# Sahar-E/NeRF-and-DietNeRF

Measured on AMD Instinct MI355X. Metric: rays/sec (coarse+fine) at 256x256, 64 coarse + 128 fine samples, higher is better.
Workload: dtype f16 (3-pass hi/lo split operands, f32 accumulate; fp32-class results)

## Files before the change

### include/nerf_mi355.h

```cpp
#ifndef NERF_MI355_H
#define NERF_MI355_H

#include <stddef.h>
#include <stdint.h>

#ifdef __cplusplus
extern "C" {
#endif

#define NERF_ABI_VERSION 6

enum { NERF_NET_COARSE = 0, NERF_NET_FINE = 1 };
enum { NERF_MEM_HOST = 0, NERF_MEM_DEVICE = 1 };
enum {
    NERF_PRECISION_FP32 = 0,
    NERF_PRECISION_F16X3 = 1,
    NERF_PRECISION_F16 = 2,
    NERF_PRECISION_BF16X3 = 3
};

enum {
    NERF_SAMPLING_LINEAR = 0,
    NERF_SAMPLING_LINDISP = 1
};
// ... 135 lines not shown
int nerf_train_render_gradients(nerf_ctx* ctx, const float* rays_orig, const float* rays_dirs, const float* d_rgb,
                                int64_t N, int32_t Sc, int32_t Sf, const float* u_coarse, const float* u_fine,
                                uint64_t seed, int64_t ray_base, int32_t accumulate, float* rgb_out,
                                float* grad_coarse, float* grad_fine, int mem);
int nerf_train_render_forward(nerf_ctx* ctx, int32_t slot, const float* rays_orig, const float* rays_dirs, int64_t N,
                              int32_t Sc, int32_t Sf, const float* u_coarse, const float* u_fine, uint64_t seed,
                              int64_t ray_base, float* rgb_out, int mem);
int nerf_train_render_backward(nerf_ctx* ctx, int32_t slot, const float* d_rgb, int32_t accumulate, float* grad_coarse,
                               float* grad_fine, int mem);
int nerf_train_render_release(nerf_ctx* ctx);
int nerf_train_get_gradients(nerf_ctx* ctx, int which, float* blob, size_t n_floats, int mem);
int nerf_get_weights(nerf_ctx* ctx, int which, float* blob, size_t n_floats, int mem);

int nerf_ctx_enable_timing(nerf_ctx* ctx, int on);
int nerf_ctx_read_timing(nerf_ctx* ctx, double* mlp_ms, int64_t* n_launches, int64_t* n_rows);
int nerf_ctx_read_culling_timing(nerf_ctx* ctx, double* ms4, int64_t* n_passes);

#ifdef __cplusplus
}
#endif
#endif
```

### nerf_and_dietnerf_amd/_lib.py

```python
from __future__ import annotations

import ctypes as C
import os

_HERE = os.path.dirname(os.path.abspath(__file__))
LIB_PATH = os.environ.get("NERF_MI355_LIB") or os.path.join(_HERE, "lib", "libnerf_mi355.so")

NERF_NET_COARSE, NERF_NET_FINE = 0, 1
NERF_MEM_HOST, NERF_MEM_DEVICE = 0, 1
NERF_PRECISION_FP32, NERF_PRECISION_F16X3, NERF_PRECISION_F16, NERF_PRECISION_BF16X3 = 0, 1, 2, 3
NERF_SAMPLING_LINEAR, NERF_SAMPLING_LINDISP = 0, 1
NERF_RAYS_WORLD, NERF_RAYS_NDC = 0, 1
NERF_ABI_VERSION = 6


class NerfConfig(C.Structure):
    _fields_ = [
        ("n_pos_enc_xyz", C.c_int32), ("n_pos_enc_dir", C.c_int32), ("n_angles", C.c_int32),
        ("hidden_dim", C.c_int32), ("last_hidden_dim", C.c_int32), ("leaky_relu_alpha", C.c_float),
        ("near_boundary", C.c_float), ("far_boundary", C.c_float), ("precision", C.c_int32),
        ("device", C.c_int32),
    ]


# ... 65 lines not shown
    ("nerf_train_set_distortion_weights", C.c_int, [_P, _F, _F]),
    ("nerf_train_read_distortion_sums", C.c_int, [_P, C.POINTER(C.c_double), C.POINTER(_I64)]),
    ("nerf_distortion_loss", C.c_int, [_P, _P, _P, _I64, _I32, _P, _P, _P, C.c_int]),
    ("nerf_train_loss_scale", C.c_int, [_P, C.POINTER(C.c_float), C.POINTER(_I64), C.POINTER(_I64)]),
    ("nerf_train_read_metric_sums", C.c_int, [_P, C.POINTER(C.c_double), C.POINTER(_I64)]),
    ("nerf_train_step", C.c_int, [_P, _P, _P, _P, _I64, _I32, _I32, _P, _P, _U64, _P, C.c_int]),
    ("nerf_train_gradients", C.c_int, [_P, _P, _P, _P, _I64, _I32, _I32, _P, _P, _U64, _P, _P, _P, C.c_int]),
    ("nerf_train_apply", C.c_int, [_P, _P, _P, C.c_int]),
    ("nerf_train_render_gradients", C.c_int, [_P, _P, _P, _P, _I64, _I32, _I32, _P, _P, _U64, _I64, _I32, _P, _P, _P,
                                              C.c_int]),
    ("nerf_train_render_forward", C.c_int, [_P, _I32, _P, _P, _I64, _I32, _I32, _P, _P, _U64, _I64, _P, C.c_int]),
    ("nerf_train_render_backward", C.c_int, [_P, _I32, _P, _I32, _P, _P, C.c_int]),
    ("nerf_train_render_release", C.c_int, [_P]),
    ("nerf_train_get_gradients", C.c_int, [_P, C.c_int, _P, C.c_size_t, C.c_int]),
    ("nerf_get_weights", C.c_int, [_P, C.c_int, _P, C.c_size_t, C.c_int]),
    ("nerf_ctx_enable_timing", C.c_int, [_P, C.c_int]),
    ("nerf_ctx_read_timing", C.c_int, [_P, C.POINTER(C.c_double), C.POINTER(_I64), C.POINTER(_I64)]),
]

_lib = None


def load():
    global _lib
    if _lib is not None:
        return _lib
    if not os.path.exists(LIB_PATH):
        raise RuntimeError(
            f"{LIB_PATH} is missing: build the HIP extension first "
            "(python -c 'import __graft_entry__ as g; g.build()' or make -C nerf_and_dietnerf_amd/csrc). "
# ... 24 lines not shown
```

### nerf_and_dietnerf_amd/csrc/mlp_f16x3.hip

```cpp
#include "mlp_f16_frag.h"

#include <math.h>
#include <string.h>

#if defined(NERF_BF16) && NERF_PE_LX == 5
namespace nerf::bf16 {
#elif defined(NERF_BF16)
namespace nerf::bf16::wide {
#elif NERF_PE_LX == 5
namespace nerf {
#else
namespace nerf::wide {
#endif

#ifdef NERF_BF16
typedef __bf16 e8 __attribute__((ext_vector_type(8)));
typedef __bf16 bf2 __attribute__((ext_vector_type(2)));
#define NERF_MFMA_E16 __builtin_amdgcn_mfma_f32_32x32x16_bf16
__device__ __forceinline__ void split_e(float y, float& hi_f, float& lo_f) {
    hi_f = __uint_as_float(__float_as_uint(y) & 0xFFFF0000u);
    lo_f = y - hi_f;
}
__device__ __forceinline__ uint32_t pack_hi(float a, float b) {
    return __builtin_amdgcn_perm(__float_as_uint(b), __float_as_uint(a), 0x07060302u);
// ... 318 lines not shown
    constexpr bool kPPBuild = false;
#else
    constexpr bool kPPBuild = true;
#endif
    constexpr bool kPP = kPPBuild && !FAST && !STASH && !XYZ;
    extern __shared__ __attribute__((aligned(16))) char smem[];
    const int tid = threadIdx.x;
    const int lane = tid & 63;
    const int wave = __builtin_amdgcn_readfirstlane(tid >> 6);
    const int j = lane & 31;
    const int h = lane >> 5;
    const uint32_t lane16 = kLdsRing + lane * 16;
    uint32_t cb_h = kLdsConst + h * 16;
    asm volatile("" : "+v"(cb_h));

    const long long ntiles = (a.M + 127) / 128;
    if ((long long)blockIdx.x >= ntiles) return;

    for (int i = tid; i < (XYZ ? kXConstFloats : kHConstFloats) / 4; i += 256) {
        const bool sig = SIGONLY && i >= kHConstBias8 / 4 && i < (kHConstBias8 + 32) / 4;
        reinterpret_cast<f32x4*>(smem + kLdsConst)[i] =
            reinterpret_cast<const f32x4*>(a.wconst)[sig ? i + (kHConstBiasSig - kHConstBias8) / 4 : i];
    }

    Pipe p;
    p.ck = 0;
    p.src_next = 0;
    p.n_chunks = XYZ ? (FAST ? kXFStreamChunks : kXStreamChunks) : SIGONLY ? kHStreamChunksSig : (FAST ? kFStreamChunks : kHStreamChunks);
    p.wbase = reinterpret_cast<const char*>(a.wstream);
    p.voff = wave * (kHCQ / 4 * kQuadBytes) + lane * 16;
    p.wave_lds = wave * (kHCQ / 4 * kQuadBytes);
    __syncthreads();
// ... 4 lines not shown
        p.src_next += 1;
#pragma unroll
        for (int j = 0; j < kHCQ / 4; ++j) dma_piece(p.cur_src, p.voff + j * kQuadBytes, p.cur_dst + j * kQuadBytes);
    }
    asm volatile("s_waitcnt vmcnt(%0)" ::"n"((kHCQ / 4) * (kHRing - 2)) : "memory");
    __builtin_amdgcn_s_barrier();
    asm volatile("" ::: "memory");

    frag4 xh[16], xl[16], nh[kPP ? 16 : 14], nl[kPP ? 16 : 14], peh[kHStepsPE], pel[kHStepsPE], dh[2], dl[2];
    f32x16 accs[4];
    float xc[64];
    float sigma_raw = 0.f;

    unsigned long long t0 = 0, t1 = 0, acc_t[8] = {0, 0, 0, 0, 0, 0, 0, 0};
    (void)t0; (void)t1; (void)acc_t;
    for (long long tile = blockIdx.x; tile < ntiles; tile += gridDim.x) {
        STAMP(t0);
        const long long m = tile * 128 + wave * 32 + j;
        const bool valid = m < a.M;
        const long long mm = valid ? m : a.M - 1;
        float px, py, pz, dx, dy, dz;
        if (a.mode == 0) {
            const long long ray = mm / a.S;
            const f32x4 o = *reinterpret_cast<const f32x4*>(a.in_a + ray * 4);
            const f32x4 d = *reinterpret_cast<const f32x4*>(a.in_b + ray * 4);
            const float zz = a.z[mm];
            px = __fadd_rn(o[0], __fmul_rn(d[0], zz));
            py = __fadd_rn(o[1], __fmul_rn(d[1], zz));
            pz = __fadd_rn(o[2], __fmul_rn(d[2], zz));
            dx = d[0]; dy = d[1]; dz = d[2];
        } else {
            px = a.in_a[mm * 3 + 0]; py = a.in_a[mm * 3 + 1]; pz = a.in_a[mm * 3 + 2];
            if constexpr (XYZ) { dx = dy = dz = 0.f; }
            else { dx = a.in_b[mm * 3 + 0]; dy = a.in_b[mm * 3 + 1]; dz = a.in_b[mm * 3 + 2]; }
        }
        const float kPi = 3.1415927410125732f;
        float pv[8 * kHStepsPE];
#pragma unroll
        for (int c = 0; c < 3; ++c) {
            const float v = c == 0 ? px : c == 1 ? py : pz;
            if constexpr (FAST) {
                sin_ladder_fp16_modes<kPeLx>(v * kPi, h, &pv[c * kPeLx]);
            } else {
#pragma unroll
                for (int k = 0; k < kPeLx; ++k) pv[c * kPeLx + k] = sin_shifted(v * (kPi * (float)(1 << k)), h);
            }
        }
        if constexpr (kPeLx == 5) {
            pv[15] = h ? 0.f : px; pv[16] = h ? 0.f : py; pv[17] = h ? 0.f : pz;
#pragma unroll
            for (int i = 18; i < 24; ++i) pv[i] = 0.f;
        } else {
            static_assert(kPeLx == 10, "the wide-PE layout holds exactly 10 octaves");
            pv[30] = h ? pz : px; pv[31] = h ? 0.f : py;
        }
#pragma unroll
        for (int n = 0; n < kHStepsPE; ++n) {
            float t8[8];
#pragma unroll
            for (int e = 0; e < 8; ++e) t8[e] = pv[n * 8 + e];
            split8<FAST>(t8, peh[n], pel[n]);
        }
        float dv[16];
#pragma unroll
        for (int c = 0; c < 3; ++c) {
            const float v = c == 0 ? dx : c == 1 ? dy : dz;
            if constexpr (FAST) {
                sin_ladder_fp16_modes<kLd>(v * kPi, h, &dv[c * kLd]);
            } else {
#pragma unroll
                for (int k = 0; k < kLd; ++k) dv[c * kLd + k] = sin_shifted(v * (kPi * (float)(1 << k)), h);
            }
        }
#pragma unroll
        for (int i = 12; i < 16; ++i) dv[i] = 0.f;
#pragma unroll
        for (int n = 0; n < 2; ++n) {
            float t8[8];
#pragma unroll
            for (int e = 0; e < 8; ++e) t8[e] = dv[n * 8 + e];
            split8<FAST>(t8, dh[n], dl[n]);
        }

        auto st_of = [&](int l) -> float* {
            if constexpr (!STASH) return nullptr;
            else {
                const long long row0 = a.diag_wrap ? (long long)(blockIdx.x & 63) * 128 + wave * 32 : tile * 128 + wave * 32;
                const long long off = row0 * (long long)a.st_ld[l] + (h * 32 + j) * 4;
                if constexpr (FAST) return reinterpret_cast<float*>(reinterpret_cast<uint16_t*>(a.st_ptr[l]) + off);
                else return a.st_ptr[l] + off;
            }
        };
        auto mk_of = [&](int l) -> frag4* {
            if constexpr (!STASH) return nullptr;
            else return a.mask_ptr[l] ? reinterpret_cast<frag4*>(a.mask_ptr[l]) + (tile * 128 + wave * 32 + j) * 2 + h
                                      : nullptr;
// ... 51 lines not shown
        } else {
            st_prev = st_cur;
            st_cur = st_of(8);
            mk_prev_ptr = mk_cur_ptr; mk_cur_ptr = mk_of(8);
            mk_prev = mk_cur; mk_cur = frag4{0u, 0u, 0u, 0u};
            if constexpr (kPP) layer_body_h<BODY_LAST, true, FAST, STASH, 0, true>(p, lane16, cb_h, kHConstBias8 * 4, a.alpha, st_prev, st_cur, mk_prev_ptr, mk_cur_ptr, mk_prev, mk_cur, accs, nh, nl, xh, xl, peh, pel, dh, dl, xc, sigma_raw);
            else layer_body_h<BODY_LAST, true, FAST, STASH>(p, lane16, cb_h, kHConstBias8 * 4, a.alpha, st_prev, st_cur, mk_prev_ptr, mk_cur_ptr, mk_prev, mk_cur, accs, xh, xl, nh, nl, peh, pel, dh, dl, xc, sigma_raw);
            STAMP(t1); acc_t[4] += t1 - t0;
        }
        if constexpr (SIGONLY) {
            if (valid && h == 0) {
                a.raw[m] = sigma_raw;
                if (a.nonfinite && !(fabsf(sigma_raw) <= 3.0e38f)) atomicAdd(a.nonfinite, 1ull);
            }
            STAMP(t0); acc_t[5] += t0 - t1; acc_t[6] += 1;
            continue;
        }
        float o0 = 0.f, o1 = 0.f, o2 = 0.f;
#pragma unroll
        for (int t = 0; t < 4; ++t) {
#pragma unroll
            for (int g = 0; g < 4; ++g) {
                constexpr int kW = XYZ ? kXConstWrgb : kHConstWrgb;
                const f32x4 w0 = lds_read4(cb_h + (kW + 0 * 128 + t * 32 + g * 8) * 4);
                const f32x4 w1 = lds_read4(cb_h + (kW + 1 * 128 + t * 32 + g * 8) * 4);
                const f32x4 w2 = lds_read4(cb_h + (kW + 2 * 128 + t * 32 + g * 8) * 4);
#pragma unroll
                for (int e = 0; e < 4; ++e) {
                    const float x = xc[t * 16 + g * 4 + e];
                    o0 = fmaf(w0[e], x, o0);
// ... 2 lines not shown
                }
            }
        }
        o0 += __shfl_xor(o0, 32);
        o1 += __shfl_xor(o1, 32);
        o2 += __shfl_xor(o2, 32);
        const f32x4 bh = lds_read4(kLdsConst + (XYZ ? kXConstBHead : kHConstBHead) * 4);
        if (valid && h == 0) {
            f32x4 out;
            out[0] = o0 + bh[0]; out[1] = o1 + bh[1]; out[2] = o2 + bh[2]; out[3] = sigma_raw;
            *reinterpret_cast<f32x4*>(a.raw + m * 4) = out;
            const float chk = out[0] + out[1] + out[2] + out[3];
            if (a.nonfinite && !(fabsf(chk) <= 3.0e38f)) atomicAdd(a.nonfinite, 1ull);
        }
        STAMP(t0); acc_t[5] += t0 - t1; acc_t[6] += 1;
    }
#ifdef NERF_STAMPS
    if (blockIdx.x == 0 && tid == 0)
        for (int i = 0; i < 8; ++i) g_stamps_h[i] = acc_t[i];
#endif
    asm volatile("s_waitcnt vmcnt(0)" ::: "memory");
}

#ifdef NERF_BF16
__global__ __launch_bounds__(256, 1) void mlp_bf16x3_kernel(const MlpArgs a) { mlp_f16_body<false>(a); }
__global__ __launch_bounds__(256, 1) void mlp_bf16x3_xyz_kernel(const MlpArgs a) { mlp_f16_body<false, false, true>(a); }
#if NERF_PE_LX == 5
__global__ __launch_bounds__(256, 1) void mlp_bf16x3_sig_kernel(const MlpArgs a) { mlp_f16_body<false, false, false, true>(a); }
#endif

// ... 36 lines not shown
__global__ __launch_bounds__(256, 1) void mlp_f16_xyz_stash_kernel(const MlpArgs a) { mlp_f16_body<true, true, true>(a); }

void launch_mlp_f16x3_stash(const MlpArgs& a, int num_cus, hipStream_t stream, bool single_pass, bool xyz_only) {
    if (a.M <= 0) return;
    const long long ntiles = (a.M + 127) / 128;
    const int grid = (int)(ntiles < (long long)num_cus ? ntiles : (long long)num_cus);
    if (xyz_only) {
        if (single_pass) hipLaunchKernelGGL(mlp_f16_xyz_stash_kernel, dim3(grid), dim3(256), kLdsTotal, stream, a);
        else hipLaunchKernelGGL(mlp_f16x3_xyz_stash_kernel, dim3(grid), dim3(256), kLdsTotal, stream, a);
        return;
    }
    if (single_pass) hipLaunchKernelGGL(mlp_f16_stash_kernel, dim3(grid), dim3(256), kLdsTotal, stream, a);
    else hipLaunchKernelGGL(mlp_f16x3_stash_kernel, dim3(grid), dim3(256), kLdsTotal, stream, a);
}

void launch_mlp_f16x3(const MlpArgs& a, int num_cus, hipStream_t stream, bool single_pass, bool xyz_only) {
    if (a.M <= 0) return;
    const long long ntiles = (a.M + 127) / 128;
    const int grid = (int)(ntiles < (long long)num_cus ? ntiles : (long long)num_cus);
    if (xyz_only) {
        if (single_pass) hipLaunchKernelGGL(mlp_f16_xyz_kernel, dim3(grid), dim3(256), kLdsTotal, stream, a);
        else hipLaunchKernelGGL(mlp_f16x3_xyz_kernel, dim3(grid), dim3(256), kLdsTotal, stream, a);
        return;
    }
    if (single_pass) hipLaunchKernelGGL(mlp_f16_kernel, dim3(grid), dim3(256), kLdsTotal, stream, a);
    else hipLaunchKernelGGL(mlp_f16x3_kernel, dim3(grid), dim3(256), kLdsTotal, stream, a);
}

#if NERF_PE_LX == 5
void launch_mlp_f16x3_sig(const MlpArgs& a, int num_cus, hipStream_t stream) {
    if (a.M <= 0) return;
    const long long ntiles = (a.M + 127) / 128;
    const int grid = (int)(ntiles < (long long)num_cus ? ntiles : (long long)num_cus);
    hipLaunchKernelGGL(mlp_f16x3_sig_kernel, dim3(grid), dim3(256), kLdsTotal, stream, a);
}
#endif

#if defined(NERF_STAMPS) && NERF_PE_LX == 5
extern "C" void nerf_debug_read_stamps_h(unsigned long long* out) {
    (void)hipDeviceSynchronize();
    (void)hipMemcpyFromSymbol(out, HIP_SYMBOL(g_stamps_h), sizeof(unsigned long long) * 16);
}
#endif

void mlp_f16x3_set_attributes() {
    (void)hipFuncSetAttribute(reinterpret_cast<const void*>(mlp_f16x3_kernel),
                              hipFuncAttributeMaxDynamicSharedMemorySize, kLdsTotal);
    (void)hipFuncSetAttribute(reinterpret_cast<const void*>(mlp_f16_kernel),
                              hipFuncAttributeMaxDynamicSharedMemorySize, kLdsTotal);
// ... 139 lines not shown
```

### nerf_and_dietnerf_amd/csrc/nerf_api.hip

```cpp
#include "../../include/nerf_mi355.h"

#include <stdarg.h>
#include <stdio.h>
#include <stdlib.h>
#include <string.h>

#include <algorithm>
#include <cmath>
#include <string>
#include <vector>

#include "nerf_ctx.h"

using namespace nerf;

thread_local std::string g_err;

namespace nerf {

int fail(const char* fmt, ...) {
    char buf[512];
    va_list ap;
    va_start(ap, fmt);
    vsnprintf(buf, sizeof buf, fmt, ap);
// ... 157 lines not shown
        if (!n.cst[d[k].cst]) HIP_OK(hipMalloc((void**)&n.cst[d[k].cst], kConstBytes));
        launch_repack(d[k].elem, dev_blob, tab, n.stream[k], d[k].bytes / (d[k].elem == kElemF32 ? 4 : 2), ctab, n.cst[d[k].cst],
                      c->stream);
    }
    HIP_OK(hipGetLastError());
    return 0;
}

}

namespace {

struct RenderKernel {
    StreamKind stream;
    ConstBlock cst;
    void (*launch)(const MlpArgs& a, int num_cus, hipStream_t s, bool xyz_only);
    bool sigma_only;
};
int pick_render_kernel(const nerf_config& cfg, int precision, bool want_sigma, RenderKernel* k) {
    const bool wide_pe = cfg.n_pos_enc_xyz > kLx, sig = want_sigma && !wide_pe && cfg.n_angles != 0;
    switch (precision) {
    case NERF_PRECISION_FP32:
        if (wide_pe)
            return fail("n_pos_enc_dim_xyz %d (> %d) renders with the 16-bit-core kernels only: precision f16x3, bf16x3 or f16, not fp32",
                        cfg.n_pos_enc_xyz, kLx);
        *k = {kFp32, kConstFp32, [](const MlpArgs& a, int n, hipStream_t s, bool x) { launch_mlp_fp32(a, n, s, x); }, false};
        return 0;
    case NERF_PRECISION_F16X3:
        if (sig) *k = {kF16x3Sig, kConst16, [](const MlpArgs& a, int n, hipStream_t s, bool) { launch_mlp_f16x3_sig(a, n, s); }, true};
        else if (wide_pe) *k = {kF16x3, kConst16, [](const MlpArgs& a, int n, hipStream_t s, bool x) { wide::launch_mlp_f16x3(a, n, s, false, x); }, false};
        else *k = {kF16x3, kConst16, [](const MlpArgs& a, int n, hipStream_t s, bool x) { launch_mlp_f16x3(a, n, s, false, x); }, false};
        return 0;
    case NERF_PRECISION_F16: {
        static const bool one_tile = [] { const char* e = getenv("NERF_F16_TILES"); return e && e[0] == '1'; }();
        if (wide_pe) *k = {kF16Hi, kConst16, [](const MlpArgs& a, int n, hipStream_t s, bool x) { wide::launch_mlp_f16x3(a, n, s, true, x); }, false};
        else if (cfg.n_angles != 0 && !one_tile) *k = {kF16Hi, kConst16, [](const MlpArgs& a, int n, hipStream_t s, bool) { launch_mlp_f16_2t(a, n, s); }, false};
        else *k = {kF16Hi, kConst16, [](const MlpArgs& a, int n, hipStream_t s, bool x) { launch_mlp_f16x3(a, n, s, true, x); }, false};
        return 0;
    }
    case NERF_PRECISION_BF16X3:
        if (sig) *k = {kBf16x3Sig, kConst16, [](const MlpArgs& a, int n, hipStream_t s, bool) { bf16::launch_mlp_bf16x3_sig(a, n, s); }, true};
        else if (wide_pe) *k = {kBf16x3, kConst16, [](const MlpArgs& a, int n, hipStream_t s, bool x) { bf16::wide::launch_mlp_bf16x3(a, n, s, x); }, false};
        else *k = {kBf16x3, kConst16, [](const MlpArgs& a, int n, hipStream_t s, bool x) { bf16::launch_mlp_bf16x3(a, n, s, x); }, false};
        return 0;
    }
    fail("unknown precision %d", precision);
    return 2;
}

int check_cfg(const nerf_config* cfg) {
    if (!cfg) return fail("nerf_config is NULL");
    if (cfg->n_angles != 2 && cfg->n_angles != 1 && cfg->n_angles != 0)
        return fail("n_angles_for_model should be 1 or 2.");
    if (cfg->n_pos_enc_xyz < 1 || cfg->n_pos_enc_xyz > kLxWide || cfg->n_pos_enc_dir < 1 || cfg->n_pos_enc_dir > kLd ||
        cfg->hidden_dim != kHidden || cfg->last_hidden_dim != kLast)
        return fail("supported networks: n_pos_enc_dim_xyz 1..%d, n_pos_enc_view_dir 1..%d, hidden %d, last hidden %d "
                    "(got %d %d %d %d)", kLxWide, kLd, kHidden, kLast, cfg->n_pos_enc_xyz, cfg->n_pos_enc_dir, cfg->hidden_dim,
                    cfg->last_hidden_dim);
// ... 3 lines not shown
                    "NERF_PRECISION_BF16X3 = 3)", cfg->precision);
    return 0;
}

int run_mlp(nerf_ctx* c, int which, const RenderKernel& k, const float* in_a, const float* in_b, const float* z, float* raw,
            long long M, int S, int mode) {
    if (!c->net[which].loaded) return fail("network %d has no weights loaded", which);
    if (int r = train_flush_weights(c, which)) return r;
    MlpArgs a{};
    a.wstream = (const float*)c->net[which].stream[k.stream];
    a.wconst = c->net[which].cst[k.cst];
    if (!a.wstream || !a.wconst) return fail("internal: network %d keeps no stream of kind %d", which, (int)k.stream);
    a.in_a = in_a; a.in_b = in_b; a.z = z; a.raw = raw; a.M = M; a.S = S; a.mode = mode;
    a.nonfinite = c->nonfinite;
    a.alpha = c->cfg.leaky_relu_alpha;
    hipEvent_t e0 = nullptr, e1 = nullptr;
    if (c->timing) {
        if (c->ev_used == c->ev_pool.size()) {
            hipEvent_t x, y;
            HIP_OK(hipEventCreate(&x));
            HIP_OK(hipEventCreate(&y));
            c->ev_pool.emplace_back(x, y);
        }
        e0 = c->ev_pool[c->ev_used].first; e1 = c->ev_pool[c->ev_used].second;
        c->ev_used++;
        c->timed_rows += M;
        HIP_OK(hipEventRecord(e0, c->stream));
    }
    k.launch(a, c->num_cus, c->stream, c->cfg.n_angles == 0);
    if (c->timing) HIP_OK(hipEventRecord(e1, c->stream));
    HIP_OK(hipGetLastError());
    return 0;
}

struct OutSizes { size_t per_ray[7]; };
OutSizes out_sizes(int S) {
    OutSizes o;
    o.per_ray[0] = 3; o.per_ray[1] = S; o.per_ray[2] = S; o.per_ray[3] = S; o.per_ray[4] = 3 * (size_t)S;
    o.per_ray[5] = S; o.per_ray[6] = 1;
    return o;
}
float** out_ptrs(nerf_outputs& o, int i) {
    switch (i) {
        case 0: return &o.rgb; case 1: return &o.weights; case 2: return &o.cumprod; case 3: return &o.alpha;
// ... 739 lines not shown
    HIP_OK(hipHostFree(p));
    return 0;
}

int nerf_ctx_read_nonfinite(nerf_ctx* c, int64_t* rows) {
    if (!c || !rows) return fail("NULL argument");
    ENTER(c);
    HIP_OK(hipStreamSynchronize(c->stream));
    unsigned long long v = 0;
    HIP_OK(hipMemcpy(&v, c->nonfinite, sizeof v, hipMemcpyDeviceToHost));
    HIP_OK(hipMemset(c->nonfinite, 0, sizeof v));
    *rows = (int64_t)v;
    return 0;
}

int nerf_ctx_enable_timing(nerf_ctx* c, int on) {
    if (!c) return fail("ctx is NULL");
    HIP_OK(hipStreamSynchronize(c->stream));
    c->timing = on != 0;
    c->ev_used = 0;
    c->cull_ev_used = 0;
    c->timed_rows = 0;
    return 0;
}

int nerf_ctx_read_timing(nerf_ctx* c, double* mlp_ms, int64_t* n_launches, int64_t* n_rows) {
    if (!c) return fail("ctx is NULL");
    HIP_OK(hipStreamSynchronize(c->stream));
    double tot = 0;
    for (size_t i = 0; i < c->ev_used; ++i) {
// ... 15 lines not shown
```

### nerf_and_dietnerf_amd/csrc/nerf_ctx.h

```cpp
#pragma once
#include "../../include/nerf_mi355.h"

#include <string>
#include <utility>
#include <vector>

#include "nerf_kernels.h"

namespace nerf {

int fail(const char* fmt, ...);

#define HIP_OK(expr)                                                                                    \
    do {                                                                                                \
        hipError_t e__ = (expr);                                                                        \
        if (e__ != hipSuccess) return nerf::fail("%s failed: %s (%s:%d)", #expr, hipGetErrorString(e__), \
                                                 __FILE__, __LINE__);                                   \
    } while (0)

struct DevBuf {
    void* p = nullptr;
    size_t cap = 0;
};

// ... 40 lines not shown
    int num_cus = 0;
    hipStream_t own_stream = nullptr;
    hipStream_t stream = nullptr;
    hipStream_t copy_stream = nullptr;
    std::vector<hipEvent_t> copy_ev;
    nerf::NetWeights net[2];
    int32_t* rt[nerf::kStreamKinds] = {};
    int32_t* rt_cst[nerf::kConstBlocks] = {};
    bool rt_built = false;
    nerf::DevBuf b_orig, b_dirs, b_zc, b_zf, b_raw, b_wc, b_u0, b_u1, b_in0, b_in1, b_in2;
    nerf::DevBuf b_out[7];
    bool timing = false;
    std::vector<std::pair<hipEvent_t, hipEvent_t>> ev_pool;
    size_t ev_used = 0;
    long long timed_rows = 0;
    unsigned long long* nonfinite = nullptr;
    nerf::TrainState* train = nullptr;
    nerf::CommState* comm = nullptr;
};

namespace nerf {

int ensure(nerf_ctx* c, DevBuf& b, size_t bytes);
int h2d(nerf_ctx* c, DevBuf& b, const void* src, size_t bytes);
int enter(nerf_ctx* c);
int copy_to_caller(nerf_ctx* c, void* dst, const void* src_dev, size_t bytes, int mem);
int copy_from_caller(nerf_ctx* c, void* dst_dev, const void* src, size_t bytes, int mem);

struct Staging {
    Staging(nerf_ctx* c, int mem);
// ... 32 lines not shown
```

### nerf_and_dietnerf_amd/csrc/nerf_kernels.h

```cpp
#pragma once
#include <hip/hip_runtime.h>
#include <stdint.h>

#include <vector>

namespace nerf {

constexpr int kLx = 5;
constexpr int kLd = 4;
constexpr int kHidden = 256;
constexpr int kLast = 128;
constexpr int kXyzDim = 3 + 6 * kLx;
constexpr int kDirDim = 6 * kLd;
int layer_dims(int lx, int ld, int n_angles, int dims[12][2]);
size_t blob_floats(int lx, int ld, int n_angles);
void blob_expand_index(int lx, int ld, int n_angles, int32_t* idx, int layout_lx = kLx);
void aim_gather(int lx, int ld, int n_angles, int32_t* idx, size_t n, bool f16);

constexpr int kQuadBytes = 1024;
constexpr int kChunkQuads = 16;
constexpr int kChunkBytes = kQuadBytes * kChunkQuads;
constexpr int kRingChunks = 8;
constexpr int kRingBytes = kChunkBytes * kRingChunks;

// ... 15 lines not shown
constexpr size_t kStreamBytesF16HiXyz = size_t(37) * 32 * kQuadBytes;

constexpr int kConstBias = 0;
constexpr int kConstBias8 = 2048;
constexpr int kConstWrgb = 2176;
constexpr int kConstBHead = 2560;
constexpr int kConstWsigH = 2564;
constexpr int kConstWsigD = 2820;
constexpr int kConstFloats = 3136;
constexpr int kConstBytes = kConstFloats * 4;

constexpr int kLdsRing = 0;
constexpr int kLdsConst = kRingBytes;
constexpr int kLdsTotal = kRingBytes + kConstBytes;

struct MlpArgs {
    const float* wstream;
    const float* wconst;
    const float* in_a;
    const float* in_b;
    const float* z;
    float* raw;
    unsigned long long* nonfinite;
    long long M;
    int S;
    int mode;
    float alpha;
    float* st_ptr[10];
    int st_ld[10];
    uint32_t* mask_ptr[10];
    int diag_wrap;
};

void launch_mlp_fp32(const MlpArgs& a, int num_cus, hipStream_t stream, bool xyz_only = false);
void mlp_fp32_set_attributes();
void build_fp32_gather(int n_angles, int32_t* stream_idx, int32_t* const_idx);

void launch_mlp_f16x3(const MlpArgs& a, int num_cus, hipStream_t stream, bool single_pass = false, bool xyz_only = false);
void launch_mlp_f16x3_stash(const MlpArgs& a, int num_cus, hipStream_t stream, bool single_pass = false, bool xyz_only = false);
void build_f16x3_gather(int n_angles, bool hi_only, int32_t* stream_idx, int32_t* const_idx);
void mlp_f16x3_set_attributes();
void launch_mlp_f16x3_sig(const MlpArgs& a, int num_cus, hipStream_t stream);
void build_f16x3_sig_gather(int n_angles, int32_t* stream_idx );

constexpr int kLxWide = 10;
namespace wide {
void launch_mlp_f16x3(const MlpArgs& a, int num_cus, hipStream_t stream, bool single_pass = false, bool xyz_only = false);
void launch_mlp_f16x3_stash(const MlpArgs& a, int num_cus, hipStream_t stream, bool single_pass = false, bool xyz_only = false);
void build_f16x3_gather(int n_angles, bool hi_only, int32_t* stream_idx, int32_t* const_idx);
void mlp_f16x3_set_attributes();
}
namespace bf16 {
void launch_mlp_bf16x3(const MlpArgs& a, int num_cus, hipStream_t stream, bool xyz_only = false);
void launch_mlp_bf16x3_sig(const MlpArgs& a, int num_cus, hipStream_t stream);
void mlp_bf16x3_set_attributes();
namespace wide {
void launch_mlp_bf16x3(const MlpArgs& a, int num_cus, hipStream_t stream, bool xyz_only = false);
void mlp_bf16x3_set_attributes();
}
}
inline int pe_layout_lx(int lx) { return lx > kLx ? kLxWide : kLx; }

// ... 100 lines not shown
```

### nerf_and_dietnerf_amd/render.py

```python
from __future__ import annotations

import ctypes as C
from typing import Dict, List, Optional, Sequence, Tuple

import numpy as np

from . import _lib
from ._lib import (NerfTrainConfig, NERF_MEM_DEVICE, NERF_MEM_HOST, NERF_NET_COARSE, NERF_NET_FINE, NERF_PRECISION_F16X3,
                   NERF_PRECISION_FP32, NerfConfig, NerfOutputs)

N_RENDER_SAMPLES_FINE = "n_render_samples_fine"
N_RENDER_SAMPLES_COARSE = "n_render_samples_coarse"
N_POS_ENC_DIM_XYZ = "n_pos_enc_dim_xyz"
N_POS_ENC_VIEW_DIR = "n_pos_enc_view_dir"
N_ANGLES_FOR_MODEL = "n_angles_for_model"
LEAKY_RELU_ALPHA = "leaky_relu_alpha"
HIDDEN_LAYER_DIM = "hidden_layer_dim"
LAST_HIDDEN_LAYER_DIM = "last_hidden_layer_dim"
N_RAYS_IN_BATCH_RENDER = "n_rays_in_batch_render"
N_RAYS_IN_BATCH_TRAIN = "n_rays_in_batch_train"
LINDISP = "lindisp"
USE_NDC = "use_ndc"
NDC_NEAR_PLANE = "ndc_near_plane"
SCENE_BOX = "scene_box"
# ... 687 lines not shown
        arr = self._arrays(grad_coarse, grad_fine)
        n = self.blob_size()
        _lib.check(self.lib.nerf_train_apply(self.h, arr.inp(grad_coarse, (n,)), arr.inp(grad_fine, (n,)), arr.mem))
        self._auto_new_weights()

    def train_get_gradients(self, which: int) -> np.ndarray:
        out = np.empty(self.blob_size(), np.float32)
        _lib.check(self.lib.nerf_train_get_gradients(self.h, which, out.ctypes.data, out.size, NERF_MEM_HOST))
        return out

    def get_weights(self, which: int) -> np.ndarray:
        out = np.empty(self.blob_size(), np.float32)
        _lib.check(self.lib.nerf_get_weights(self.h, which, out.ctypes.data, out.size, NERF_MEM_HOST))
        return out

    def enable_timing(self, on: bool = True) -> None:
        _lib.check(self.lib.nerf_ctx_enable_timing(self.h, int(on)))

    def read_timing(self) -> Tuple[float, int, int]:
        ms, n, rows = C.c_double(), C.c_int64(), C.c_int64()
        _lib.check(self.lib.nerf_ctx_read_timing(self.h, C.byref(ms), C.byref(n), C.byref(rows)))
        return ms.value, n.value, rows.value

    def _arrays(self, *probe) -> "_Arrays":
        arr = _Arrays(*probe)
        if arr.torch is not None:
            cur = arr.torch.cuda.current_stream(arr.device).cuda_stream
            if cur != self._stream:
                _lib.check(self.lib.nerf_ctx_set_stream(self.h, C.c_void_p(cur)))
                self._stream = cur
# ... 462 lines not shown
```

Before: 1.712 million.

## Process runs of samples per ray to reuse direction encoding in f16x3 MLP

Adds a run-based row ordering to the f16x3 MLP kernels. Each lane handles a run of consecutive samples from the same ray across several tiles, so the ray origin/direction load and the view-direction encoding and split are done once per run instead of once per sample, and the next z value is prefetched. A host-side planner picks the run length and only uses runs in auto mode when the per-CU work does not grow beyond the canonical tiling. The change adds goto-based loop control, a new MlpArgs layout, and API calls to force or count the mode. In exchange it raises register pressure and changes the row-to-lane mapping and load coalescing.

```diff
diff --git a/include/nerf_mi355.h b/include/nerf_mi355.h
--- a/include/nerf_mi355.h
+++ b/include/nerf_mi355.h
@@ -173,6 +173,11 @@
 
 int nerf_ctx_enable_timing(nerf_ctx* ctx, int on);
 int nerf_ctx_read_timing(nerf_ctx* ctx, double* mlp_ms, int64_t* n_launches, int64_t* n_rows);
+#define NERF_ROW_ORDER_AUTO 0
+#define NERF_ROW_ORDER_CANONICAL 1
+#define NERF_ROW_ORDER_RUNS 2
+int nerf_ctx_set_row_order(nerf_ctx* ctx, int mode);
+int nerf_ctx_row_order_counts(nerf_ctx* ctx, int64_t* run_launches, int64_t* canonical_launches);
 int nerf_ctx_read_culling_timing(nerf_ctx* ctx, double* ms4, int64_t* n_passes);
 
 #ifdef __cplusplus
diff --git a/nerf_and_dietnerf_amd/_lib.py b/nerf_and_dietnerf_amd/_lib.py
--- a/nerf_and_dietnerf_amd/_lib.py
+++ b/nerf_and_dietnerf_amd/_lib.py
@@ -103,6 +103,8 @@
     ("nerf_train_render_release", C.c_int, [_P]),
     ("nerf_train_get_gradients", C.c_int, [_P, C.c_int, _P, C.c_size_t, C.c_int]),
     ("nerf_get_weights", C.c_int, [_P, C.c_int, _P, C.c_size_t, C.c_int]),
+    ("nerf_ctx_set_row_order", C.c_int, [_P, C.c_int]),
+    ("nerf_ctx_row_order_counts", C.c_int, [_P, C.POINTER(_I64), C.POINTER(_I64)]),
     ("nerf_ctx_enable_timing", C.c_int, [_P, C.c_int]),
     ("nerf_ctx_read_timing", C.c_int, [_P, C.POINTER(C.c_double), C.POINTER(_I64), C.POINTER(_I64)]),
 ]
diff --git a/nerf_and_dietnerf_amd/csrc/mlp_f16x3.hip b/nerf_and_dietnerf_amd/csrc/mlp_f16x3.hip
--- a/nerf_and_dietnerf_amd/csrc/mlp_f16x3.hip
+++ b/nerf_and_dietnerf_amd/csrc/mlp_f16x3.hip
@@ -356,8 +356,14 @@
     uint32_t cb_h = kLdsConst + h * 16;
     asm volatile("" : "+v"(cb_h));
 
-    const long long ntiles = (a.M + 127) / 128;
+    const bool runs = kPP && a.run_tiles > 0;
+    const int T = runs ? a.run_tiles : 1;
+    const long long n_rays = runs ? a.M / a.S : 0;
+    const int run_q = runs ? (a.S >> a.run_lk) / T : 1;
+    const long long run_count = runs ? ((n_rays + (32 >> a.run_lk) - 1) >> (5 - a.run_lk)) * run_q : 0;
+    const long long ntiles = runs ? (run_count + 3) / 4 : (a.M + 127) / 128;
     if ((long long)blockIdx.x >= ntiles) return;
+    (void)T; (void)n_rays; (void)run_q;
 
     for (int i = tid; i < (XYZ ? kXConstFloats : kHConstFloats) / 4; i += 256) {
         const bool sig = SIGONLY && i >= kHConstBias8 / 4 && i < (kHConstBias8 + 32) / 4;
@@ -392,12 +398,93 @@
 
     unsigned long long t0 = 0, t1 = 0, acc_t[8] = {0, 0, 0, 0, 0, 0, 0, 0};
     (void)t0; (void)t1; (void)acc_t;
+    const float kPi = 3.1415927410125732f;
+    auto encode_dirs = [&](float dx, float dy, float dz) {
+        float dv[16];
+#pragma unroll
+        for (int c = 0; c < 3; ++c) {
+            const float v = c == 0 ? dx : c == 1 ? dy : dz;
+            if constexpr (FAST) {
+                sin_ladder_fp16_modes<kLd>(v * kPi, h, &dv[c * kLd]);
+            } else {
+#pragma unroll
+                for (int k = 0; k < kLd; ++k) dv[c * kLd + k] = sin_shifted(v * (kPi * (float)(1 << k)), h);
+            }
+        }
+#pragma unroll
+        for (int i = 12; i < 16; ++i) dv[i] = 0.f;
+#pragma unroll
+        for (int n = 0; n < 2; ++n) {
+            float t8[8];
+#pragma unroll
+            for (int e = 0; e < 8; ++e) t8[e] = dv[n * 8 + e];
+            split8<FAST>(t8, dh[n], dl[n]);
+        }
+    };
     for (long long tile = blockIdx.x; tile < ntiles; tile += gridDim.x) {
         STAMP(t0);
-        const long long m = tile * 128 + wave * 32 + j;
-        const bool valid = m < a.M;
+        long long row = 0;
+        int row_step = 0;
+        bool run_valid = false;
+        float ox = 0.f, oy = 0.f, oz = 0.f, rx = 0.f, ry = 0.f, rz = 0.f, z_next = 0.f;
+        (void)row_step; (void)run_valid; (void)ox; (void)oy; (void)oz; (void)rx; (void)ry; (void)rz; (void)z_next;
+        if constexpr (kPP) {
+            long long ray = 0;
+            if (runs) {
+                const long long r = tile * 4 + wave;
+                const long long rc = r < run_count ? r : run_count - 1;
+                const long long g = rc / run_q;
+                const int q = (int)(rc - g * run_q);
+                const int K = 1 << a.run_lk;
+                const long long lane_ray = g * (32 >> a.run_lk) + (j >> a.run_lk);
+                run_valid = r < run_count && lane_ray < n_rays;
+                ray = lane_ray < n_rays ? lane_ray : n_rays - 1;
+                row = ray * a.S + (long long)q * T * K + (j & (K - 1));
+                row_step = K;
+            } else {
+                const long long m0 = tile * 128 + wave * 32 + j;
+                run_valid = m0 < a.M;
+                row = run_valid ? m0 : a.M - 1;
+                if (a.mode == 0) ray = row / a.S;
+            }
+            if (a.mode == 0) {
+                const f32x4 o = *reinterpret_cast<const f32x4*>(a.in_a + ray * 4);
+                const f32x4 d = *reinterpret_cast<const f32x4*>(a.in_b + ray * 4);
+                z_next = a.z[row];
+                ox = o[0]; oy = o[1]; oz = o[2];
+                rx = d[0]; ry = d[1]; rz = d[2];
+            } else {
+                rx = a.in_b[row * 3 + 0]; ry = a.in_b[row * 3 + 1]; rz = a.in_b[row * 3 + 2];
+            }
+            encode_dirs(rx, ry, rz);
+        }
+        int t = 0;
+        (void)t;
+    next_tile:
+        long long m;
+        bool valid;
+        float px, py, pz;
+        if constexpr (kPP) {
+            m = row;
+            valid = run_valid;
+            if (a.mode == 0) {
+                const float zz = z_next;
+                if (t + 1 < T) z_next = a.z[row + row_step];
+                px = __fadd_rn(ox, __fmul_rn(rx, zz));
+                py = __fadd_rn(oy, __fmul_rn(ry, zz));
+                pz = __fadd_rn(oz, __fmul_rn(rz, zz));
+            } else {
+                px = a.in_a[row * 3 + 0]; py = a.in_a[row * 3 + 1]; pz = a.in_a[row * 3 + 2];
+            }
+            row += row_step;
+        } else {
+            m = tile * 128 + wave * 32 + j;
+            valid = m < a.M;
+        }
+        float dx = 0.f, dy = 0.f, dz = 0.f;
+        (void)dx; (void)dy; (void)dz;
+        if constexpr (!kPP) {
         const long long mm = valid ? m : a.M - 1;
-        float px, py, pz, dx, dy, dz;
         if (a.mode == 0) {
             const long long ray = mm / a.S;
             const f32x4 o = *reinterpret_cast<const f32x4*>(a.in_a + ray * 4);
@@ -412,7 +499,7 @@
             if constexpr (XYZ) { dx = dy = dz = 0.f; }
             else { dx = a.in_b[mm * 3 + 0]; dy = a.in_b[mm * 3 + 1]; dz = a.in_b[mm * 3 + 2]; }
         }
-        const float kPi = 3.1415927410125732f;
+        }
         float pv[8 * kHStepsPE];
 #pragma unroll
         for (int c = 0; c < 3; ++c) {
@@ -439,6 +526,7 @@
             for (int e = 0; e < 8; ++e) t8[e] = pv[n * 8 + e];
             split8<FAST>(t8, peh[n], pel[n]);
         }
+        if constexpr (!kPP) {
         float dv[16];
 #pragma unroll
         for (int c = 0; c < 3; ++c) {
@@ -458,6 +546,7 @@
 #pragma unroll
             for (int e = 0; e < 8; ++e) t8[e] = dv[n * 8 + e];
             split8<FAST>(t8, dh[n], dl[n]);
+        }
         }
 
         auto st_of = [&](int l) -> float* {
@@ -539,6 +628,7 @@
                 if (a.nonfinite && !(fabsf(sigma_raw) <= 3.0e38f)) atomicAdd(a.nonfinite, 1ull);
             }
             STAMP(t0); acc_t[5] += t0 - t1; acc_t[6] += 1;
+            if constexpr (kPP) { if (++t < T) goto next_tile; }
             continue;
         }
         float o0 = 0.f, o1 = 0.f, o2 = 0.f;
@@ -571,6 +661,7 @@
             if (a.nonfinite && !(fabsf(chk) <= 3.0e38f)) atomicAdd(a.nonfinite, 1ull);
         }
         STAMP(t0); acc_t[5] += t0 - t1; acc_t[6] += 1;
+        if constexpr (kPP) { if (++t < T) goto next_tile; }
     }
 #ifdef NERF_STAMPS
     if (blockIdx.x == 0 && tid == 0)
@@ -637,25 +728,51 @@
     else hipLaunchKernelGGL(mlp_f16x3_stash_kernel, dim3(grid), dim3(256), kLdsTotal, stream, a);
 }
 
-void launch_mlp_f16x3(const MlpArgs& a, int num_cus, hipStream_t stream, bool single_pass, bool xyz_only) {
-    if (a.M <= 0) return;
+static long long plan_rows(MlpArgs& a, int num_cus, int kmax_lk) {
+    const long long tiles = (a.M + 127) / 128;
+    a.run_tiles = 0; a.run_lk = 0;
+#if NERF_PE_LX == 5
+    if (a.mode != 0 || a.row_order == kRowOrderCanonical || a.S <= 0 || a.M % a.S != 0) return tiles;
+    const long long n_rays = a.M / a.S, G = num_cus;
+    int lk = kmax_lk;
+    if (a.row_order == kRowOrderRuns) while (a.S % (1 << lk)) --lk;
+    else if (a.S % (1 << lk)) return tiles;
+    const int per_group = a.S >> lk;
+    const long long groups = (n_rays + (32 >> lk) - 1) / (32 >> lk);
+    for (int T = per_group; T >= 1; --T) {
+        if (per_group % T) continue;
+        const long long steps = (groups * (per_group / T) + 3) / 4;
+        if (a.row_order != kRowOrderRuns && (steps + G - 1) / G * T > (tiles + G - 1) / G) continue;
+        a.run_tiles = T; a.run_lk = (int16_t)lk;
+        return steps;
+    }
+#endif
+    return tiles;
+}
+
+bool launch_mlp_f16x3(const MlpArgs& a, int num_cus, hipStream_t stream, bool single_pass, bool xyz_only) {
+    if (a.M <= 0) return false;
     const long long ntiles = (a.M + 127) / 128;
     const int grid = (int)(ntiles < (long long)num_cus ? ntiles : (long long)num_cus);
     if (xyz_only) {
         if (single_pass) hipLaunchKernelGGL(mlp_f16_xyz_kernel, dim3(grid), dim3(256), kLdsTotal, stream, a);
         else hipLaunchKernelGGL(mlp_f16x3_xyz_kernel, dim3(grid), dim3(256), kLdsTotal, stream, a);
-        return;
-    }
-    if (single_pass) hipLaunchKernelGGL(mlp_f16_kernel, dim3(grid), dim3(256), kLdsTotal, stream, a);
-    else hipLaunchKernelGGL(mlp_f16x3_kernel, dim3(grid), dim3(256), kLdsTotal, stream, a);
+        return false;
+    }
+    if (single_pass) { hipLaunchKernelGGL(mlp_f16_kernel, dim3(grid), dim3(256), kLdsTotal, stream, a); return false; }
+    MlpArgs b = a;
+    const long long steps = plan_rows(b, num_cus, 5);
+    hipLaunchKernelGGL(mlp_f16x3_kernel, dim3((int)(steps < (long long)num_cus ? steps : (long long)num_cus)), dim3(256), kLdsTotal, stream, b);
+    return b.run_tiles > 0;
 }
 
 #if NERF_PE_LX == 5
-void launch_mlp_f16x3_sig(const MlpArgs& a, int num_cus, hipStream_t stream) {
-    if (a.M <= 0) return;
-    const long long ntiles = (a.M + 127) / 128;
-    const int grid = (int)(ntiles < (long long)num_cus ? ntiles : (long long)num_cus);
-    hipLaunchKernelGGL(mlp_f16x3_sig_kernel, dim3(grid), dim3(256), kLdsTotal, stream, a);
+bool launch_mlp_f16x3_sig(const MlpArgs& a, int num_cus, hipStream_t stream) {
+    if (a.M <= 0) return false;
+    MlpArgs b = a;
+    const long long steps = plan_rows(b, num_cus, 4);
+    hipLaunchKernelGGL(mlp_f16x3_sig_kernel, dim3((int)(steps < (long long)num_cus ? steps : (long long)num_cus)), dim3(256), kLdsTotal, stream, b);
+    return b.run_tiles > 0;
 }
 #endif
 
diff --git a/nerf_and_dietnerf_amd/csrc/nerf_api.hip b/nerf_and_dietnerf_amd/csrc/nerf_api.hip
--- a/nerf_and_dietnerf_amd/csrc/nerf_api.hip
+++ b/nerf_and_dietnerf_amd/csrc/nerf_api.hip
@@ -195,7 +195,7 @@
 struct RenderKernel {
     StreamKind stream;
     ConstBlock cst;
-    void (*launch)(const MlpArgs& a, int num_cus, hipStream_t s, bool xyz_only);
+    bool (*launch)(const MlpArgs& a, int num_cus, hipStream_t s, bool xyz_only);
     bool sigma_only;
 };
 int pick_render_kernel(const nerf_config& cfg, int precision, bool want_sigma, RenderKernel* k) {
@@ -205,24 +205,24 @@
         if (wide_pe)
             return fail("n_pos_enc_dim_xyz %d (> %d) renders with the 16-bit-core kernels only: precision f16x3, bf16x3 or f16, not fp32",
                         cfg.n_pos_enc_xyz, kLx);
-        *k = {kFp32, kConstFp32, [](const MlpArgs& a, int n, hipStream_t s, bool x) { launch_mlp_fp32(a, n, s, x); }, false};
+        *k = {kFp32, kConstFp32, [](const MlpArgs& a, int n, hipStream_t s, bool x) { launch_mlp_fp32(a, n, s, x); return false; }, false};
         return 0;
     case NERF_PRECISION_F16X3:
-        if (sig) *k = {kF16x3Sig, kConst16, [](const MlpArgs& a, int n, hipStream_t s, bool) { launch_mlp_f16x3_sig(a, n, s); }, true};
-        else if (wide_pe) *k = {kF16x3, kConst16, [](const MlpArgs& a, int n, hipStream_t s, bool x) { wide::launch_mlp_f16x3(a, n, s, false, x); }, false};
-        else *k = {kF16x3, kConst16, [](const MlpArgs& a, int n, hipStream_t s, bool x) { launch_mlp_f16x3(a, n, s, false, x); }, false};
+        if (sig) *k = {kF16x3Sig, kConst16, [](const MlpArgs& a, int n, hipStream_t s, bool) { return launch_mlp_f16x3_sig(a, n, s); }, true};
+        else if (wide_pe) *k = {kF16x3, kConst16, [](const MlpArgs& a, int n, hipStream_t s, bool x) { return wide::launch_mlp_f16x3(a, n, s, false, x); }, false};
+        else *k = {kF16x3, kConst16, [](const MlpArgs& a, int n, hipStream_t s, bool x) { return launch_mlp_f16x3(a, n, s, false, x); }, false};
         return 0;
     case NERF_PRECISION_F16: {
         static const bool one_tile = [] { const char* e = getenv("NERF_F16_TILES"); return e && e[0] == '1'; }();
-        if (wide_pe) *k = {kF16Hi, kConst16, [](const MlpArgs& a, int n, hipStream_t s, bool x) { wide::launch_mlp_f16x3(a, n, s, true, x); }, false};
-        else if (cfg.n_angles != 0 && !one_tile) *k = {kF16Hi, kConst16, [](const MlpArgs& a, int n, hipStream_t s, bool) { launch_mlp_f16_2t(a, n, s); }, false};
-        else *k = {kF16Hi, kConst16, [](const MlpArgs& a, int n, hipStream_t s, bool x) { launch_mlp_f16x3(a, n, s, true, x); }, false};
+        if (wide_pe) *k = {kF16Hi, kConst16, [](const MlpArgs& a, int n, hipStream_t s, bool x) { return wide::launch_mlp_f16x3(a, n, s, true, x); }, false};
+        else if (cfg.n_angles != 0 && !one_tile) *k = {kF16Hi, kConst16, [](const MlpArgs& a, int n, hipStream_t s, bool) { launch_mlp_f16_2t(a, n, s); return false; }, false};
+        else *k = {kF16Hi, kConst16, [](const MlpArgs& a, int n, hipStream_t s, bool x) { return launch_mlp_f16x3(a, n, s, true, x); }, false};
         return 0;
     }
     case NERF_PRECISION_BF16X3:
-        if (sig) *k = {kBf16x3Sig, kConst16, [](const MlpArgs& a, int n, hipStream_t s, bool) { bf16::launch_mlp_bf16x3_sig(a, n, s); }, true};
-        else if (wide_pe) *k = {kBf16x3, kConst16, [](const MlpArgs& a, int n, hipStream_t s, bool x) { bf16::wide::launch_mlp_bf16x3(a, n, s, x); }, false};
-        else *k = {kBf16x3, kConst16, [](const MlpArgs& a, int n, hipStream_t s, bool x) { bf16::launch_mlp_bf16x3(a, n, s, x); }, false};
+        if (sig) *k = {kBf16x3Sig, kConst16, [](const MlpArgs& a, int n, hipStream_t s, bool) { bf16::launch_mlp_bf16x3_sig(a, n, s); return false; }, true};
+        else if (wide_pe) *k = {kBf16x3, kConst16, [](const MlpArgs& a, int n, hipStream_t s, bool x) { bf16::wide::launch_mlp_bf16x3(a, n, s, x); return false; }, false};
+        else *k = {kBf16x3, kConst16, [](const MlpArgs& a, int n, hipStream_t s, bool x) { bf16::launch_mlp_bf16x3(a, n, s, x); return false; }, false};
         return 0;
     }
     fail("unknown precision %d", precision);
@@ -256,6 +256,7 @@
     a.in_a = in_a; a.in_b = in_b; a.z = z; a.raw = raw; a.M = M; a.S = S; a.mode = mode;
     a.nonfinite = c->nonfinite;
     a.alpha = c->cfg.leaky_relu_alpha;
+    a.row_order = c->row_order;
     hipEvent_t e0 = nullptr, e1 = nullptr;
     if (c->timing) {
         if (c->ev_used == c->ev_pool.size()) {
@@ -269,7 +270,7 @@
         c->timed_rows += M;
         HIP_OK(hipEventRecord(e0, c->stream));
     }
-    k.launch(a, c->num_cus, c->stream, c->cfg.n_angles == 0);
+    if (M > 0) (k.launch(a, c->num_cus, c->stream, c->cfg.n_angles == 0) ? c->run_launches : c->canonical_launches)++;
     if (c->timing) HIP_OK(hipEventRecord(e1, c->stream));
     HIP_OK(hipGetLastError());
     return 0;
@@ -1039,6 +1040,23 @@
     return 0;
 }
 
+int nerf_ctx_set_row_order(nerf_ctx* c, int mode) {
+    if (!c) return fail("ctx is NULL");
+    static_assert(NERF_ROW_ORDER_AUTO == kRowOrderAuto && NERF_ROW_ORDER_CANONICAL == kRowOrderCanonical &&
+                  NERF_ROW_ORDER_RUNS == kRowOrderRuns, "the launchers read these values");
+    if (mode != NERF_ROW_ORDER_AUTO && mode != NERF_ROW_ORDER_CANONICAL && mode != NERF_ROW_ORDER_RUNS)
+        return fail("row order %d: NERF_ROW_ORDER_AUTO = 0, NERF_ROW_ORDER_CANONICAL = 1, NERF_ROW_ORDER_RUNS = 2", mode);
+    c->row_order = mode;
+    return 0;
+}
+
+int nerf_ctx_row_order_counts(nerf_ctx* c, int64_t* run_launches, int64_t* canonical_launches) {
+    if (!c) return fail("ctx is NULL");
+    if (run_launches) *run_launches = c->run_launches;
+    if (canonical_launches) *canonical_launches = c->canonical_launches;
+    return 0;
+}
+
 int nerf_ctx_enable_timing(nerf_ctx* c, int on) {
     if (!c) return fail("ctx is NULL");
     HIP_OK(hipStreamSynchronize(c->stream));
diff --git a/nerf_and_dietnerf_amd/csrc/nerf_ctx.h b/nerf_and_dietnerf_amd/csrc/nerf_ctx.h
--- a/nerf_and_dietnerf_amd/csrc/nerf_ctx.h
+++ b/nerf_and_dietnerf_amd/csrc/nerf_ctx.h
@@ -78,6 +78,8 @@
     std::vector<std::pair<hipEvent_t, hipEvent_t>> ev_pool;
     size_t ev_used = 0;
     long long timed_rows = 0;
+    int row_order = 0;
+    long long run_launches = 0, canonical_launches = 0;
     unsigned long long* nonfinite = nullptr;
     nerf::TrainState* train = nullptr;
     nerf::CommState* comm = nullptr;
diff --git a/nerf_and_dietnerf_amd/csrc/nerf_kernels.h b/nerf_and_dietnerf_amd/csrc/nerf_kernels.h
--- a/nerf_and_dietnerf_amd/csrc/nerf_kernels.h
+++ b/nerf_and_dietnerf_amd/csrc/nerf_kernels.h
@@ -53,6 +53,7 @@
 constexpr int kLdsConst = kRingBytes;
 constexpr int kLdsTotal = kRingBytes + kConstBytes;
 
+enum { kRowOrderAuto = 0, kRowOrderCanonical = 1, kRowOrderRuns = 2 };
 struct MlpArgs {
     const float* wstream;
     const float* wconst;
@@ -65,26 +66,29 @@
     int S;
     int mode;
     float alpha;
+    int run_tiles;
     float* st_ptr[10];
     int st_ld[10];
     uint32_t* mask_ptr[10];
     int diag_wrap;
+    int16_t run_lk, row_order;
 };
+static_assert(sizeof(MlpArgs) == 288, "run_tiles, run_lk and row_order fill padding");
 
 void launch_mlp_fp32(const MlpArgs& a, int num_cus, hipStream_t stream, bool xyz_only = false);
 void mlp_fp32_set_attributes();
 void build_fp32_gather(int n_angles, int32_t* stream_idx, int32_t* const_idx);
 
-void launch_mlp_f16x3(const MlpArgs& a, int num_cus, hipStream_t stream, bool single_pass = false, bool xyz_only = false);
+bool launch_mlp_f16x3(const MlpArgs& a, int num_cus, hipStream_t stream, bool single_pass = false, bool xyz_only = false);
 void launch_mlp_f16x3_stash(const MlpArgs& a, int num_cus, hipStream_t stream, bool single_pass = false, bool xyz_only = false);
 void build_f16x3_gather(int n_angles, bool hi_only, int32_t* stream_idx, int32_t* const_idx);
 void mlp_f16x3_set_attributes();
-void launch_mlp_f16x3_sig(const MlpArgs& a, int num_cus, hipStream_t stream);
+bool launch_mlp_f16x3_sig(const MlpArgs& a, int num_cus, hipStream_t stream);
 void build_f16x3_sig_gather(int n_angles, int32_t* stream_idx );
 
 constexpr int kLxWide = 10;
 namespace wide {
-void launch_mlp_f16x3(const MlpArgs& a, int num_cus, hipStream_t stream, bool single_pass = false, bool xyz_only = false);
+bool launch_mlp_f16x3(const MlpArgs& a, int num_cus, hipStream_t stream, bool single_pass = false, bool xyz_only = false);
 void launch_mlp_f16x3_stash(const MlpArgs& a, int num_cus, hipStream_t stream, bool single_pass = false, bool xyz_only = false);
 void build_f16x3_gather(int n_angles, bool hi_only, int32_t* stream_idx, int32_t* const_idx);
 void mlp_f16x3_set_attributes();
diff --git a/nerf_and_dietnerf_amd/render.py b/nerf_and_dietnerf_amd/render.py
--- a/nerf_and_dietnerf_amd/render.py
+++ b/nerf_and_dietnerf_amd/render.py
@@ -725,6 +725,14 @@
         _lib.check(self.lib.nerf_get_weights(self.h, which, out.ctypes.data, out.size, NERF_MEM_HOST))
         return out
 
+    def set_row_order(self, mode: int) -> None:
+        _lib.check(self.lib.nerf_ctx_set_row_order(self.h, int(mode)))
+
+    def row_order_counts(self) -> Tuple[int, int]:
+        runs, canon = C.c_int64(), C.c_int64()
+        _lib.check(self.lib.nerf_ctx_row_order_counts(self.h, C.byref(runs), C.byref(canon)))
+        return runs.value, canon.value
+
     def enable_timing(self, on: bool = True) -> None:
         _lib.check(self.lib.nerf_ctx_enable_timing(self.h, int(on)))
 
```

Result: no change. 1.726 million, median of 6 (+0.8%).
